# facebookresearch/sam-audio

Hardware: AMD Instinct MI355X
Metric: seconds-of-audio separated/sec/node (higher is better)
Workload: dtype fp16x3 (fp32 storage as the reference; every big contraction on IEEE-half hi + lo split operands: 3 MFMA products per multiply, fp32 accumulation - fp32-grade results on the 16-bit matrix cores)

## Files before the change

### include/samaudio.h

```cpp
#ifndef SAMAUDIO_H_
#define SAMAUDIO_H_

#include <stddef.h>
#include <stdint.h>

#ifdef __cplusplus
extern "C" {
#endif

typedef struct samaudio_ctx samaudio_ctx;
typedef void* samaudio_stream;

enum { SAMAUDIO_F32 = 0, SAMAUDIO_BF16 = 1 };
enum { SAMAUDIO_DT_F32 = 0, SAMAUDIO_DT_BF16 = 1, SAMAUDIO_DT_I64 = 2, SAMAUDIO_DT_U8 = 3 };
enum { SAMAUDIO_ODE_EULER = 0, SAMAUDIO_ODE_MIDPOINT = 1, SAMAUDIO_ODE_RK4 = 2, SAMAUDIO_ODE_HEUN3 = 3 };

enum {
  SAMAUDIO_OK = 0,
  SAMAUDIO_ERR_ARG = -1,
  SAMAUDIO_ERR_WEIGHT = -2,
  SAMAUDIO_ERR_WORKSPACE = -3,
  SAMAUDIO_ERR_HIP = -4,
  SAMAUDIO_ERR_STATE = -5
};
// ... 269 lines not shown
                                      int dim, float eps, samaudio_stream stream);
int samaudio_op_split3(const float* x, int64_t x_ld, void* out, int64_t rows, int k, samaudio_stream stream);


int samaudio_op_mod_tables(const float* const* w, const float* const* shift_tab, const float* const* scale_tab,
                           const int* shift_off, const int* scale_off, int n_norms, const float* tvec, int64_t tvec_ld,
                           int n_time, float* gs, int dim, samaudio_stream stream);
int samaudio_op_rmsnorm_gs(const float* x, const float* gs, int64_t gs_ld, void* out, int precision, int form, int rows,
                           int dim, int rows_per_batch, float eps, samaudio_stream stream);
int samaudio_op_qkv_prep_hd(const void* qkv, const float* q_w, const float* k_w, const float* rope_cos,
                            const float* rope_sin, void* q, void* k, void* vt, int precision, int form, int batch,
                            int frames, int frames_padded, int heads, int head_dim, float eps, samaudio_stream stream);
int samaudio_op_self_attention_hd(const void* q, const void* k, const void* vt, const uint8_t* key_mask, void* out,
                                  int precision, int form, int batch, int frames, int frames_padded, int heads,
                                  int head_dim, samaudio_stream stream);
int samaudio_op_cross_attention_hd(const void* q, const float* q_w, void* kv, int64_t kv_ld, const float* k_w,
                                   const uint8_t* mask, void* out, int precision, int batch, int frames, int text_len,
                                   int heads, int head_dim, float eps, samaudio_stream stream);
int samaudio_op_cross_attn_probs(const void* q, const float* q_w, const void* kv, int64_t kv_ld, const uint8_t* mask, void* p,
                                 int ldp, int batch, int frames, int text_len, int ltp, int heads, float eps,
                                 samaudio_stream stream);
int samaudio_op_cross_attn_probs3(const float* q, const float* q_w, const float* kv, int64_t kv_ld, const uint8_t* mask, void* p3,
                                  int kp, int batch, int frames, int text_len, int ltp, int heads, float eps,
                                  samaudio_stream stream);
int samaudio_op_cross_attn_fold3(const float* wo, const float* kv, int64_t kv_ld, void* ut3, int kp, int batch, int text_len,
                                 int ltp, int heads, samaudio_stream stream);

#ifdef __cplusplus
}
#endif
// ... 2 lines not shown
```

### sam_audio_amd/csrc/api.hip

```cpp
#include <cstring>
#include <string>

#include "engine.h"
#include "peav.h"

struct samaudio_ctx {
  sa::Engine* engine;
};
struct samaudio_judge {
  sa::Judge* judge;
};
struct samaudio_frame {
  sa::FramePredictor* frame;
};

namespace {
thread_local std::string g_err;
}
namespace sa {
void set_last_error(const std::string& msg) { g_err = msg; }
}
namespace {
int hip_ret(hipError_t e, const char* what) {
  if (e == hipSuccess) return SAMAUDIO_OK;
// ... 335 lines not shown
  if (form == 1 && !bf16) return bad("rmsnorm_gs: the alt-16 form belongs to 16-bit contexts");
  return hip_ret(sa::launch_rmsnorm_gs(x, gs, gs_ld, out, bf16, rows, dim, rows_per_batch, eps, (hipStream_t)stream, form == 1),
                 "rmsnorm_gs");
}

int samaudio_op_qkv_prep_hd(const void* qkv, const float* q_w, const float* k_w, const float* rope_cos,
                            const float* rope_sin, void* q, void* k, void* vt, int precision, int form, int batch,
                            int frames, int frames_padded, int heads, int head_dim, float eps, samaudio_stream stream) {
  if (frames_padded % 64 || frames_padded < frames || frames <= 0) return bad("qkv_prep_hd: frames_padded");
  if (head_dim != 64 && head_dim != 128) return bad("qkv_prep_hd: head_dim");
  if (form == 1) {
    if (precision != SAMAUDIO_F32 || head_dim != 128) return bad("qkv_prep_hd: the f32x form takes fp32 tensors and head_dim 128");
    return hip_ret(sa::launch_qkv_prep_f32x((const float*)qkv, q_w, k_w, rope_cos, rope_sin, (float*)q, (float*)k, (float*)vt, batch,
                                            frames, frames_padded, heads, eps, (hipStream_t)stream), "qkv_prep_f32x");
  }
  if (form != 0) return bad("qkv_prep_hd: form");
  return hip_ret(sa::launch_qkv_prep(qkv, q_w, k_w, rope_cos, rope_sin, q, k, vt, precision == SAMAUDIO_BF16, batch, frames,
                                     frames_padded, heads, eps, (hipStream_t)stream, head_dim), "qkv_prep");
}

int samaudio_op_self_attention_hd(const void* q, const void* k, const void* vt, const uint8_t* key_mask, void* out,
                                  int precision, int form, int batch, int frames, int frames_padded, int heads,
                                  int head_dim, samaudio_stream stream) {
  if (frames_padded % 64 || frames_padded < frames || frames <= 0) return bad("self_attention_hd: frames_padded");
  if (head_dim != 64 && head_dim != 128) return bad("self_attention_hd: head_dim");
  if (precision < 0 || precision > 2 || form < 0 || form > 2) return bad("self_attention_hd: precision / form");
  if (form == 1 && precision != SAMAUDIO_BF16) return bad("self_attention_hd: the alt-16 output belongs to the 16-bit kernel");
  if (form == 2 && precision != 2) return bad("self_attention_hd: the split output belongs to the compensated kernel");
  if (precision == 2)
    return hip_ret(sa::launch_self_attention_x3((const float*)q, (const float*)k, (const float*)vt, key_mask,
                                                form == 2 ? nullptr : (float*)out, batch, frames, frames_padded, heads, head_dim,
                                                (hipStream_t)stream, form == 2 ? out : nullptr), "self_attention_x3");
  return hip_ret(sa::launch_self_attention_hd(q, k, vt, key_mask, out, precision == SAMAUDIO_BF16, batch, frames, frames_padded,
                                              heads, head_dim, (hipStream_t)stream, form == 1), "self_attention_hd");
}

int samaudio_op_cross_attention_hd(const void* q, const float* q_w, void* kv, int64_t kv_ld, const float* k_w,
                                   const uint8_t* mask, void* out, int precision, int batch, int frames, int text_len,
                                   int heads, int head_dim, float eps, samaudio_stream stream) {
  if (head_dim != 64 && head_dim != 128) return bad("cross_attention_hd: head_dim");
  if (batch <= 0 || frames <= 0 || text_len <= 0 || heads <= 0 || kv_ld < 2L * heads * head_dim || kv_ld % 8)
    return bad("cross_attention_hd: shape / kv_ld");
  const bool bf16 = precision == SAMAUDIO_BF16;
  hipError_t e = sa::launch_headnorm(kv, k_w, bf16, batch * text_len, kv_ld, 0, heads, eps, (hipStream_t)stream, head_dim);
  if (e != hipSuccess) return hip_ret(e, "headnorm");
  return hip_ret(sa::launch_cross_attention(q, q_w, kv, kv_ld, mask, out, bf16, batch, frames, text_len, heads, eps,
                                            (hipStream_t)stream, head_dim), "cross_attention");
}

int samaudio_op_cross_attn_probs(const void* q, const float* q_w, const void* kv, int64_t kv_ld, const uint8_t* mask, void* p,
                                 int ldp, int batch, int frames, int text_len, int ltp, int heads, float eps,
// ... 122 lines not shown
```

### sam_audio_amd/csrc/attention.hip

```cpp
#include "kernels.h"

namespace sa {

typedef h16x8_t bf16x8_t;
typedef __attribute__((ext_vector_type(4))) float f32x4_t;

template <int NW, int HD, bool OUT_ALT = false>
__global__ __launch_bounds__(NW * 64, 4) void self_attn_bf16_kernel(const bf16_t* __restrict__ Q, const bf16_t* __restrict__ K,
                                                                 const bf16_t* __restrict__ Vt,
                                                                 const unsigned char* __restrict__ key_mask,
                                                                 bf16_t* __restrict__ out, int T, int Tp, int H) {
  constexpr int CH = HD / 8;
  constexpr int KS = HD / 32;
  constexpr int NF = HD / 16;
  __shared__ __attribute__((aligned(16))) char Ks[64 * HD * 2];
  __shared__ __attribute__((aligned(16))) char Vs[HD * 128];
  __shared__ __attribute__((aligned(16))) char Ps[NW * 16 * 128];
  const int qb = blockIdx.x, h = blockIdx.y, b = blockIdx.z;
  const int q0 = qb * (16 * NW);
  const int tid = threadIdx.x, lane = tid & 63, wave = tid >> 6;
  const int lr = lane & 15, lg = lane >> 4;
  const long bh = (long)b * H + h;
  const float scale = HD == 128 ? 0.08838834764831845f : 0.125f;

// ... 399 lines not shown
        bf16_t* dst = out3 + ((long)b * T + q) * (3L * D) + h * HD + c * 8;
        *(uint4*)dst = lo;
        *(uint4*)(dst + D) = hi;
        *(uint4*)(dst + 2L * D) = hi;
      }
    }
    return;
  }
  constexpr int CPRO = HD / 4;
#pragma unroll
  for (int u = lane; u < 16 * CPRO; u += 64) {
    const int row = u / CPRO, c = u % CPRO;
    const int q = q0 + wave * 16 + row;
    if (q < T) *(uint4*)(out + ((long)b * T + q) * D + h * HD + c * 4) = *(const uint4*)(mine + row * (HD * 4) + c * 16);
  }
}

template <int HD>
static hipError_t launch_self_attention_t(const void* Q, const void* K, const void* Vt, const unsigned char* key_mask,
                                          void* out, bool bf16, int B, int T, int Tp, int H, hipStream_t st, bool out_alt = false) {
  if (bf16 && out_alt && Tp % 128 == 0)
    hipLaunchKernelGGL((self_attn_bf16_kernel<8, HD, true>), dim3(Tp / 128, H, B), dim3(512), 0, st, (const bf16_t*)Q, (const bf16_t*)K,
                       (const bf16_t*)Vt, key_mask, (bf16_t*)out, T, Tp, H);
  else if (bf16 && out_alt)
    hipLaunchKernelGGL((self_attn_bf16_kernel<4, HD, true>), dim3(Tp / 64, H, B), dim3(256), 0, st, (const bf16_t*)Q, (const bf16_t*)K,
                       (const bf16_t*)Vt, key_mask, (bf16_t*)out, T, Tp, H);
  else if (out_alt)
    return hipErrorInvalidValue;
  else if (bf16 && Tp % 128 == 0)
    hipLaunchKernelGGL((self_attn_bf16_kernel<8, HD>), dim3(Tp / 128, H, B), dim3(512), 0, st, (const bf16_t*)Q, (const bf16_t*)K,
// ... 605 lines not shown
```

### sam_audio_amd/csrc/engine.h

```cpp
#pragma once
#include "host.h"

namespace sa {

constexpr int HALO = 40;

class Engine {
 public:
  explicit Engine(const samaudio_config& c);
  Status set_tensor(const char* name, const void* p, int dtype, int ndim, const int64_t* shape);
  Status finalize(int what);
  Status set_option(int option, int value);
  Status check_f32_weights(int classes) const;
  size_t workspace_bytes(int rows, int frames, int text_len, int codec_items, int64_t samples);
  Status set_workspace(void* p, size_t bytes);

  Status prepare(int rows, int frames, int text_len, const float* feats, const float* text, const uint8_t* text_mask,
                 const float* video, const int64_t* anchor_ids, int n_ids, const int64_t* anchor_alignment,
                 const uint8_t* pad_mask, hipStream_t st, int candidates = 1, bool latent_feats = false);
  Status forward(const float* noisy, const float* time, int n_time, float* out, hipStream_t st);
  Status ode_solve(float* state, int method, const float* grid_host, int n_grid, hipStream_t st);
  struct RkTableau;
  size_t ode_stage_bytes(int method, int rows, int frames) const;
  Status set_ode_stages(void* p, size_t bytes);
// ... 44 lines not shown
  bool f32c(int cls) const { return bf16_ && (f32_classes_ & cls) != 0; }
  bool alt16(int cls) const { return bf16_ && (alt_classes_ & cls) != 0; }
  const void* opt(const std::string& name, std::vector<int64_t> shape) const;
  struct ProfRec {
    std::string key;
    double flops, bytes;
    hipEvent_t e0, e1;
  };
  template <class F>
  Status op(const char* name, double alg_bytes, double alg_flops, hipStream_t st, F&& launch);
  Status res_unit(GemmParams p, GemmParams q, void*& cur, void*& alt, double flops7, double flops1, hipStream_t st);
  struct SBuf;
  struct StageW;
  Status res_units(const StageW& sw, SBuf& sb, int n, const float* next_alpha, hipStream_t st);
  void* hash_ = nullptr;
  bool prof_on_ = false;
  std::vector<ProfRec> prof_;
  std::vector<hipEvent_t> ev_pool_;
  size_t ev_used_ = 0;
  Status prof_event(hipEvent_t* e);

  samaudio_config cfg_;
  bool bf16_;
  bool tail_split_ = true;
  int f32_classes_ = 0;
  int alt_classes_ = 0;
  int prefetch_rows_ = 0;
  int x3_classes_ = 0;
  Status solve_launches(float* y, int method, const float* grid, int n_grid, hipStream_t st);
  Status solve_rk(float* y, const RkTableau& tab, const float* grid, int n_grid, hipStream_t st);
// ... 62 lines not shown
```

### sam_audio_amd/csrc/engine.hip

```cpp
#include "engine.h"

#include <algorithm>
#include <cmath>
#include <cstdio>
#include <cstdlib>
#include <cstring>

namespace sa {

static bool trace_on() {
  static const bool on = std::getenv("SAMAUDIO_TRACE") != nullptr;
  return on;
}
struct HashTrace {
  struct Rec { std::string name; int items; size_t slot; };
  unsigned long long* dev = nullptr;
  size_t used = 0, seq = 0;
  std::vector<Rec> recs;
  static constexpr size_t CAP = 1 << 20;
  bool full_warned = false;
};
struct HashScope {
  explicit HashScope(HashTrace* h, int items);
  ~HashScope();
// ... 55 lines not shown
#else
      const unsigned u = (unsigned)((const unsigned short*)host.data())[i] << 16;
      std::memcpy(&v, &u, 4);
#endif
    } else {
      v = ((const float*)host.data())[i];
    }
    if (!std::isfinite(v)) ++bad;
    else if (std::fabs(v) > mx) mx = std::fabs(v);
  }
  std::fprintf(stderr, "[samaudio trace] %-22s n=%zu non-finite=%zu max|x|=%.4g\n", name, count, bad, mx);
}

Engine::Engine(const samaudio_config& c) : cfg_(c) {
  bf16_ = c.precision == SAMAUDIO_BF16;
  esz_ = bf16_ ? 2 : 4;
  at_dtype_ = bf16_ ? SAMAUDIO_DT_BF16 : SAMAUDIO_DT_F32;
  std::memset(&g32_, 0, sizeof(g32_));
  std::memset(&enc_, 0, sizeof(enc_));
  std::memset(&dec_, 0, sizeof(dec_));
  std::memset(&d_, 0, sizeof(d_));
}

Status Registry::set(const char* name, const void* p, int dtype, int ndim, const int64_t* shape) {
  if (!name || !p || ndim < 0 || ndim > 4) return fail(SAMAUDIO_ERR_ARG, "set_tensor: bad argument");
  if ((reinterpret_cast<uintptr_t>(p) & 15) != 0)
    return fail(SAMAUDIO_ERR_ARG, std::string("set_tensor: ") + name + " is not 16-byte aligned");
  TensorRef t;
  t.p = p;
  t.dtype = dtype;
// ... 1004 lines not shown
    return p;
  };
  for (int l = 0; l < cfg_.n_layers; ++l) {
    const LayerW& w = layers_[l];
    const float* tab = w.mod_table;
    const bool qkv_pre = x3(SAMAUDIO_CLS_QKV) && mod_gs, w13_pre = x3(SAMAUDIO_CLS_W13) && mod_gs;
    const bool wo_pre = x3(SAMAUDIO_CLS_WO) && x3(SAMAUDIO_X3_ATTENTION);
    bool w2_pre = false;
    SA_TRY(norm_for(l, 0, SAMAUDIO_CLS_QKV, qkv_pre));
    {
      GemmParams p = lin(d_.xn, D, nullptr, M, 3 * D, D);
      prefetch(p, w.wo.w, (double)D * D);
      out_act(p, d_.qkv, 3L * D);
      SA_TRY(linear(p, w.wqkv, SAMAUDIO_CLS_QKV, st, qkv_pre ? d_.x3a : nullptr));
    }
    SA_TRY(op("qkv_prep", 2 * 3 * MD * esz_, 0, st, [&] {
      if (x3(SAMAUDIO_X3_ATTENTION) && hd == 128)
        return launch_qkv_prep_f32x((const float*)d_.qkv, w.q_norm, w.k_norm, g_.rope_cos, g_.rope_sin, (float*)d_.Q, (float*)d_.K,
                                    (float*)d_.Vt, rows, T, Tp, H, eps, st);
      return launch_qkv_prep(d_.qkv, w.q_norm, w.k_norm, g_.rope_cos, g_.rope_sin, d_.Q, d_.K, d_.Vt, bf16_, rows, T, Tp, H,
                             eps, st, hd);
    }));
    trace("  xn", d_.xn, (size_t)M * D, bf16_, st);
    trace("  qkv", d_.qkv, (size_t)M * 3 * D, bf16_, st);
    trace("  Q", d_.Q, (size_t)rows * Tp * D, bf16_, st);
    trace("  K", d_.K, (size_t)rows * Tp * D, bf16_, st);
    trace("  Vt", d_.Vt, (size_t)rows * Tp * D, bf16_, st);
    if (x3(SAMAUDIO_X3_ATTENTION))
      SA_TRY(op("self_attention_x3", 4 * MD * 4, 4.0 * T * T * D * rows, st, [&] {
        return launch_self_attention_x3((const float*)d_.Q, (const float*)d_.K, (const float*)d_.Vt, d_.pad_mask, (float*)d_.attn, rows,
                                        T, Tp, H, hd, st, wo_pre ? d_.x3a : nullptr);
      }));
    else
    SA_TRY(op("self_attention", 4 * MD * esz_, 4.0 * T * T * D * rows, st, [&] {
      return launch_self_attention_hd(d_.Q, d_.K, d_.Vt, d_.pad_mask, d_.attn, bf16_, rows, T, Tp, H, hd, st, alt16(SAMAUDIO_CLS_WO));
    }));
    trace("  attn", d_.attn, (size_t)M * D, bf16_, st);
    SA_TRY(sentinel(15, d_.attn, !bf16_ ? 0 : (alt16(SAMAUDIO_CLS_WO) ? 2 : 1), M, D, D, st));
    {
      GemmParams p = lin(d_.attn, D, nullptr, M, D, D);
      p.gate_tab = tab + 2 * D; p.gate = d_.t0 + 2 * D; p.gate_ld = t6; p.rows_per_gate = T;
      with_res(p, d_.h, D);
      out_f32(p, d_.h, D);
      out_act(p, d_.hbf, D);
// ... 370 lines not shown
```

### sam_audio_amd/csrc/kernels.h

```cpp
#pragma once
#include "common.h"

namespace sa {

hipError_t launch_poison_lds(hipStream_t st);

enum DebugFlag : int {
  DBG_NO_CONV7H = 11,
  DBG_RESUNIT_TWO_LAUNCHES = 16,
  DBG_RESUNIT_FUSE_ALWAYS = 18,
  DBG_RESUNIT_WS = 19,
  DBG_GEMM8S_PLAIN = 21,
  DBG_GEMM8_EPILOGUE = 24,
  DBG_GEMM8_NOT_PERSISTENT = 26,
  DBG_GEMM8S_ROLES = 27,
  DBG_QKV_PREP_SWROUND = 29,
  DBG_GEMM8_MIN_TILES = 30,
  DBG_FOLD_PER_LAYER = 31,
  DBG_TAIL_SPLIT_MIN = 33,
  DBG_RASTER_GM = 35,
  DBG_FLY_OLD_TILES = 36,
  DBG_X3_PLAIN_WALK = 38,
};
enum : int { DBG_WS_ALWAYS = 1, DBG_WS_NEVER = 2, DBG_WS_ALWAYS_GRID3 = 3 };
// ... 108 lines not shown
                           float eps, hipStream_t st, int head_dim = 128);

hipError_t launch_qkv_prep_f32x(const float* qkv, const float* qw, const float* kw, const float* rope_cos, const float* rope_sin, float* Q,
                                float* K, float* Vt, int B, int T, int Tp, int H, float eps, hipStream_t st);

hipError_t launch_self_attention(const void* Q, const void* K, const void* Vt, const unsigned char* key_mask,
                                 void* out, bool bf16, int B, int T, int Tp, int H, hipStream_t st, bool out_alt = false);

hipError_t launch_self_attention_hd(const void* Q, const void* K, const void* Vt, const unsigned char* key_mask,
                                    void* out, bool bf16, int B, int T, int Tp, int H, int head_dim, hipStream_t st,
                                    bool out_alt = false);

hipError_t launch_self_attention_x3(const float* Q, const float* K, const float* Vt, const unsigned char* key_mask, float* out,
                                    int B, int T, int Tp, int H, int head_dim, hipStream_t st, void* out3 = nullptr);

hipError_t launch_headnorm(void* x, const float* w, bool bf16, int rows, long ld, int col0, int H, float eps,
                           hipStream_t st, int head_dim = 128);

hipError_t launch_cross_attention(const void* q, const float* qw, const void* kv, long kv_ld,
                                  const unsigned char* mask, void* out, bool bf16, int B, int T, int Lt, int H,
                                  float eps, hipStream_t st, int head_dim = 128);
hipError_t launch_cross_attn_probs(const void* q, const float* qw, const void* kv, long kv_ld, const unsigned char* mask,
                                   void* P, int ldp, int B, int T, int Lt, int LtP, int H, float eps, hipStream_t st);
hipError_t launch_cross_attn_fold(const void* wo, const void* kv, long kv_ld, void* UT, int KP, int B, int Lt, int LtP,
                                  int H, hipStream_t st);
constexpr int kMaxFoldLayers = 48;
hipError_t launch_cross_attn_fold_layers(const void* const* wo, int n_layers, const void* kv_all, long kv_ld, void* UT_all, int KP,
                                         int B, int Lt, int LtP, int H, hipStream_t st);
hipError_t launch_cross_attn_probs3(const float* q, const float* qw, const float* kv, long kv_ld, const unsigned char* mask, void* P3,
                                    int KP, int B, int T, int Lt, int LtP, int H, float eps, hipStream_t st);
// ... 83 lines not shown
```

### sam_audio_amd/csrc/kernels.hip

```cpp
#include "kernels.h"

namespace sa {

static int g_debug_flags[64] = {0};
void set_debug_flag(int flag, int value) {
  if (flag >= 0 && flag < 64) g_debug_flags[flag] = value;
}
int debug_flag(int flag) { return flag >= 0 && flag < 64 ? g_debug_flags[flag] : 0; }

template <typename TO>
__global__ __launch_bounds__(256) void rmsnorm_mod_kernel(const float* __restrict__ x, const float* __restrict__ w,
                                                          const float* __restrict__ shift_tab,
                                                          const float* __restrict__ scale_tab,
                                                          const float* __restrict__ tvec, long tvec_ld, int shift_off,
                                                          int scale_off, TO* __restrict__ out, int M, int D,
                                                          int rows_per_b, float eps) {
  const int row = blockIdx.x * 4 + (threadIdx.x >> 6);
  if (row >= M) return;
  const int lane = threadIdx.x & 63;
  const float4* xr = (const float4*)(x + (long)row * D);
  const int n4 = D >> 2;
  float ss = 0.f;
  for (int i = lane; i < n4; i += 64) {
    float4 v = xr[i];
// ... 427 lines not shown
  }
  __syncthreads();
#pragma unroll
  for (int it = 0; it < 4; ++it) {
    const int item = it * 256 + tid;
    const int d = item >> 3, c = item & 7;
    unsigned short x[8];
#pragma unroll
    for (int e = 0; e < 8; ++e) x[e] = vt[(c * 8 + e) * 136 + d];
    const uint4 o = make_uint4((unsigned)x[0] | ((unsigned)x[1] << 16), (unsigned)x[2] | ((unsigned)x[3] << 16),
                               (unsigned)x[4] | ((unsigned)x[5] << 16), (unsigned)x[6] | ((unsigned)x[7] << 16));
    *(uint4*)(Vt + (bh * 128 + d) * Tp + t0 + c * 8) = o;
  }
}

__global__ __launch_bounds__(256) void qkv_prep_f32x_kernel(const float* __restrict__ qkv, const float* __restrict__ qw,
                                                            const float* __restrict__ kw, const float* __restrict__ rc,
                                                            const float* __restrict__ rs, float* __restrict__ Q, float* __restrict__ K,
                                                            float* __restrict__ Vt, int T, int Tp, int H, float eps) {
  __shared__ __attribute__((aligned(16))) float vt[64 * 132];
  const int t0 = blockIdx.x * 64, h = blockIdx.y, b = blockIdx.z;
  const int D = H * 128;
  const long ld = 3L * D;
  const int tid = threadIdx.x;
  const int sub = tid & 15;
  const int rgrp = tid >> 4;
  const long bh = (long)b * H + h;
  float wq[8], wk[8];
  {
    const float4 a = *(const float4*)(qw + sub * 8), c = *(const float4*)(qw + sub * 8 + 4);
    const float4 e = *(const float4*)(kw + sub * 8), f = *(const float4*)(kw + sub * 8 + 4);
    wq[0] = a.x; wq[1] = a.y; wq[2] = a.z; wq[3] = a.w; wq[4] = c.x; wq[5] = c.y; wq[6] = c.z; wq[7] = c.w;
    wk[0] = e.x; wk[1] = e.y; wk[2] = e.z; wk[3] = e.w; wk[4] = f.x; wk[5] = f.y; wk[6] = f.z; wk[7] = f.w;
  }
#pragma unroll
// ... 15 lines not shown
      sq = row16_sum(sq);
      sk = row16_sum(sk);
      const float iq = rsqrtf(sq / 128.f + eps), ik = rsqrtf(sk / 128.f + eps);
      const float4 c4 = *(const float4*)(rc + (long)t * 64 + sub * 4), s4 = *(const float4*)(rs + (long)t * 64 + sub * 4);
      const float cc[4] = {c4.x, c4.y, c4.z, c4.w}, sn[4] = {s4.x, s4.y, s4.z, s4.w};
#pragma unroll
      for (int e = 0; e < 4; ++e) {
        const float a0 = q[2 * e] * iq * wq[2 * e], a1 = q[2 * e + 1] * iq * wq[2 * e + 1];
        q[2 * e] = a0 * cc[e] - a1 * sn[e];
        q[2 * e + 1] = a0 * sn[e] + a1 * cc[e];
        const float b0 = k[2 * e] * ik * wk[2 * e], b1 = k[2 * e + 1] * ik * wk[2 * e + 1];
        k[2 * e] = b0 * cc[e] - b1 * sn[e];
        k[2 * e + 1] = b0 * sn[e] + b1 * cc[e];
      }
    }
    float* qd = Q + (bh * Tp + t) * 128 + sub * 8;
    float* kd = K + (bh * Tp + t) * 128 + sub * 8;
    *(float4*)qd = make_float4(q[0], q[1], q[2], q[3]);
    *(float4*)(qd + 4) = make_float4(q[4], q[5], q[6], q[7]);
    *(float4*)kd = make_float4(k[0], k[1], k[2], k[3]);
    *(float4*)(kd + 4) = make_float4(k[4], k[5], k[6], k[7]);
    *(float4*)(vt + tt * 132 + sub * 8) = v0;
    *(float4*)(vt + tt * 132 + sub * 8 + 4) = v1;
  }
  __syncthreads();
#pragma unroll
  for (int it = 0; it < 4; ++it) {
    const int item = it * 256 + tid;
    const int d = item >> 3, c = item & 7;
    float x[8];
#pragma unroll
    for (int e = 0; e < 8; ++e) x[e] = vt[(c * 8 + e) * 132 + d];
    float* dst = Vt + (bh * 128 + d) * Tp + t0 + c * 8;
    *(float4*)dst = make_float4(x[0], x[1], x[2], x[3]);
    *(float4*)(dst + 4) = make_float4(x[4], x[5], x[6], x[7]);
  }
}
hipError_t launch_qkv_prep_f32x(const float* qkv, const float* qw, const float* kw, const float* rope_cos, const float* rope_sin, float* Q,
                                float* K, float* Vt, int B, int T, int Tp, int H, float eps, hipStream_t st) {
  if (Tp % 64) return hipErrorInvalidValue;
  hipLaunchKernelGGL(qkv_prep_f32x_kernel, dim3(Tp / 64, H, B), dim3(256), 0, st, qkv, qw, kw, rope_cos, rope_sin, Q, K, Vt, T, Tp, H, eps);
  return hipGetLastError();
}

hipError_t launch_qkv_prep(const void* qkv, const float* qw, const float* kw, const float* rope_cos,
                           const float* rope_sin, void* Q, void* K, void* Vt, bool bf16, int B, int T, int Tp, int H,
                           float eps, hipStream_t st, int head_dim) {
  dim3 grid(Tp / 64, H, B), block(256);
  if (head_dim == 64) {
    if (bf16)
      hipLaunchKernelGGL((qkv_prep_kernel<bf16_t, 64>), grid, block, 0, st, (const bf16_t*)qkv, qw, kw, rope_cos, rope_sin, (bf16_t*)Q,
                         (bf16_t*)K, (bf16_t*)Vt, T, Tp, H, eps);
    else
      hipLaunchKernelGGL((qkv_prep_kernel<float, 64>), grid, block, 0, st, (const float*)qkv, qw, kw, rope_cos, rope_sin, (float*)Q,
                         (float*)K, (float*)Vt, T, Tp, H, eps);
    return hipGetLastError();
// ... 506 lines not shown
```

### sam_audio_amd/hip.py

```python
from __future__ import annotations

import ctypes as C
import os
import threading
from typing import Optional, Sequence

_HERE = os.path.dirname(os.path.abspath(__file__))
LIB_PATH = os.path.join(_HERE, "libsamaudio_hip.so")
LIB_PATHS = {"bf16": LIB_PATH, "fp16": os.path.join(_HERE, "libsamaudio_hip_f16.so")}

F32, BF16 = 0, 1
DT_F32, DT_BF16, DT_I64, DT_U8 = 0, 1, 2, 3
PRECISIONS = ("bf16", "fp16", "mixed", "fp32")
X3_PRECISIONS = ("fp16x3", "bf16x3")


def check_precision(precision: str, x3_ok: bool = False) -> None:
    if precision not in PRECISIONS + (X3_PRECISIONS if x3_ok else ()):
        raise ValueError("precision must be 'bf16', 'fp16', 'mixed' or 'fp32'" + (", 'fp16x3' or 'bf16x3'" if x3_ok else ""))


def is_x3(precision: str) -> bool:
    return precision in X3_PRECISIONS

# ... 226 lines not shown
    "samaudio_op_self_attention": (C.c_int, [C.c_void_p] * 5 + [C.c_int] * 5 + [C.c_void_p]),
    "samaudio_op_cross_attention": (C.c_int, [C.c_void_p] * 6 + [C.c_int] * 5 + [C.c_float, C.c_void_p]),
    "samaudio_op_cross_attn_fold": (C.c_int, [C.c_void_p, C.c_void_p, C.c_int64, C.c_void_p] + [C.c_int] * 5 + [C.c_void_p]),
    "samaudio_op_layernorm_accum": (C.c_int, [C.c_void_p] * 5 + [C.c_int, C.c_int, C.c_float, C.c_void_p]),
    "samaudio_op_masked_groupnorm_silu": (C.c_int, [C.c_void_p] * 6 + [C.c_int] * 5 + [C.c_float, C.c_void_p]),
    "samaudio_op_masked_groupnorm_silu_split3": (C.c_int, [C.c_void_p] * 6 + [C.c_int] * 4 + [C.c_float, C.c_void_p]),
    "samaudio_op_layernorm_rows": (C.c_int, [C.c_void_p, C.c_int64] + [C.c_void_p] * 4 + [C.c_int, C.c_int64, C.c_int,
                                                                                          C.c_float, C.c_void_p]),
    "samaudio_op_layernorm_rows_split3": (C.c_int, [C.c_void_p, C.c_int64] + [C.c_void_p] * 3 + [C.c_int64, C.c_int, C.c_float, C.c_void_p]),
    "samaudio_op_split3": (C.c_int, [C.c_void_p, C.c_int64, C.c_void_p, C.c_int64, C.c_int, C.c_void_p]),
    "samaudio_op_mod_tables": (C.c_int, [C.POINTER(C.c_void_p)] * 3 + [C.POINTER(C.c_int)] * 2 + [C.c_int, C.c_void_p, C.c_int64,
                                                                                                 C.c_int, C.c_void_p, C.c_int, C.c_void_p]),
    "samaudio_op_rmsnorm_gs": (C.c_int, [C.c_void_p, C.c_void_p, C.c_int64, C.c_void_p] + [C.c_int] * 5 + [C.c_float, C.c_void_p]),
    "samaudio_op_qkv_prep_hd": (C.c_int, [C.c_void_p] * 8 + [C.c_int] * 7 + [C.c_float, C.c_void_p]),
    "samaudio_op_self_attention_hd": (C.c_int, [C.c_void_p] * 5 + [C.c_int] * 7 + [C.c_void_p]),
    "samaudio_op_cross_attention_hd": (C.c_int, [C.c_void_p] * 3 + [C.c_int64] + [C.c_void_p] * 3 + [C.c_int] * 6 + [C.c_float, C.c_void_p]),
    "samaudio_op_cross_attn_probs": (C.c_int, [C.c_void_p] * 3 + [C.c_int64, C.c_void_p, C.c_void_p] + [C.c_int] * 6 + [C.c_float, C.c_void_p]),
    "samaudio_op_cross_attn_probs3": (C.c_int, [C.c_void_p] * 3 + [C.c_int64, C.c_void_p, C.c_void_p] + [C.c_int] * 6 + [C.c_float, C.c_void_p]),
    "samaudio_op_cross_attn_fold3": (C.c_int, [C.c_void_p, C.c_void_p, C.c_int64, C.c_void_p] + [C.c_int] * 5 + [C.c_void_p]),
    "samaudio_judge_create": (C.c_int, [C.POINTER(JudgeConfig), C.POINTER(C.c_void_p)]),
    "samaudio_judge_destroy": (None, [C.c_void_p]),
    "samaudio_judge_set_tensor": (C.c_int, [C.c_void_p, C.c_char_p, C.c_void_p, C.c_int, C.c_int, C.POINTER(C.c_int64)]),
    "samaudio_judge_set_option": (C.c_int, [C.c_void_p, C.c_int, C.c_int]),
    "samaudio_judge_finalize": (C.c_int, [C.c_void_p]),
    "samaudio_judge_workspace_bytes": (C.c_size_t, [C.c_void_p, C.c_int, C.c_int, C.c_int]),
    "samaudio_judge_set_workspace": (C.c_int, [C.c_void_p, C.c_void_p, C.c_size_t]),
    "samaudio_judge_score": (C.c_int, [C.c_void_p, C.c_void_p, C.c_void_p, C.c_int, C.c_int, C.c_int, C.c_void_p,
                                       C.c_void_p, C.c_void_p, C.c_void_p]),
    "samaudio_judge_encode": (C.c_int, [C.c_void_p, C.c_int, C.c_void_p, C.c_void_p, C.c_int, C.c_int, C.c_void_p,
                                        C.c_void_p]),
# ... 101 lines not shown
```

Measured before the change: 95.23.

## Pre-split Q/K/V into hi/lo 16-bit planes for compensated self-attention

The qkv prep kernel gains a planes mode that writes Q, K and V^T as separate high and low 16-bit planes instead of fp32. A new self-attention kernel reads these planes directly, staging K and V^T in LDS through register prefetch, and runs the three-product split MFMAs without re-splitting fp32 operands inside the loop. The goal is to halve attention operand traffic and remove the per-tile split work. It adds weak-symbol dispatch and an environment opt-out, and it depends on the split done at prep time matching the accuracy of the old path.

```diff
diff --git a/include/samaudio.h b/include/samaudio.h
--- a/include/samaudio.h
+++ b/include/samaudio.h
@@ -307,6 +307,8 @@
 int samaudio_op_self_attention_hd(const void* q, const void* k, const void* vt, const uint8_t* key_mask, void* out,
                                   int precision, int form, int batch, int frames, int frames_padded, int heads,
                                   int head_dim, samaudio_stream stream);
+int samaudio_op_self_attention_planes(const void* q, const void* k, const void* vt, const uint8_t* key_mask, void* out, int form,
+                                      int batch, int frames, int frames_padded, int heads, samaudio_stream stream);
 int samaudio_op_cross_attention_hd(const void* q, const float* q_w, void* kv, int64_t kv_ld, const float* k_w,
                                    const uint8_t* mask, void* out, int precision, int batch, int frames, int text_len,
                                    int heads, int head_dim, float eps, samaudio_stream stream);
diff --git a/sam_audio_amd/csrc/api.hip b/sam_audio_amd/csrc/api.hip
--- a/sam_audio_amd/csrc/api.hip
+++ b/sam_audio_amd/csrc/api.hip
@@ -373,6 +373,17 @@
     return hip_ret(sa::launch_qkv_prep_f32x((const float*)qkv, q_w, k_w, rope_cos, rope_sin, (float*)q, (float*)k, (float*)vt, batch,
                                             frames, frames_padded, heads, eps, (hipStream_t)stream), "qkv_prep_f32x");
   }
+  if (form == 2) {
+    if (precision != SAMAUDIO_F32 || head_dim != 128) return bad("qkv_prep_hd: the planes form takes fp32 tensors and head_dim 128");
+    if (!qkv || !q_w || !k_w || !rope_cos || !rope_sin || !q || !k || !vt || batch <= 0 || heads <= 0)
+      return bad("qkv_prep_hd: null argument / batch, heads");
+    if (!sa::launch_qkv_prep_planes) {
+      g_err = "qkv_prep_hd: the planes form is not in this build of the library";
+      return SAMAUDIO_ERR_STATE;
+    }
+    return hip_ret(sa::launch_qkv_prep_planes((const float*)qkv, q_w, k_w, rope_cos, rope_sin, q, k, vt, batch, frames, frames_padded,
+                                              heads, eps, (hipStream_t)stream), "qkv_prep_planes");
+  }
   if (form != 0) return bad("qkv_prep_hd: form");
   return hip_ret(sa::launch_qkv_prep(qkv, q_w, k_w, rope_cos, rope_sin, q, k, vt, precision == SAMAUDIO_BF16, batch, frames,
                                      frames_padded, heads, eps, (hipStream_t)stream, head_dim), "qkv_prep");
@@ -394,6 +405,19 @@
                                               heads, head_dim, (hipStream_t)stream, form == 1), "self_attention_hd");
 }
 
+int samaudio_op_self_attention_planes(const void* q, const void* k, const void* vt, const uint8_t* key_mask, void* out, int form,
+                                      int batch, int frames, int frames_padded, int heads, samaudio_stream stream) {
+  if (!q || !k || !vt || !key_mask || !out || batch <= 0 || heads <= 0) return bad("self_attention_planes: null argument / batch, heads");
+  if (frames_padded % 64 || frames_padded < frames || frames <= 0) return bad("self_attention_planes: frames_padded");
+  if (form != 0 && form != 2) return bad("self_attention_planes: form");
+  if (!sa::launch_self_attention_x3p) {
+    g_err = "self_attention_planes: not in this build of the library";
+    return SAMAUDIO_ERR_STATE;
+  }
+  return hip_ret(sa::launch_self_attention_x3p(q, k, vt, key_mask, form == 2 ? nullptr : (float*)out, batch, frames, frames_padded, heads,
+                                               (hipStream_t)stream, form == 2 ? out : nullptr), "self_attention_x3p");
+}
+
 int samaudio_op_cross_attention_hd(const void* q, const float* q_w, void* kv, int64_t kv_ld, const float* k_w,
                                    const uint8_t* mask, void* out, int precision, int batch, int frames, int text_len,
                                    int heads, int head_dim, float eps, samaudio_stream stream) {
diff --git a/sam_audio_amd/csrc/attention.hip b/sam_audio_amd/csrc/attention.hip
--- a/sam_audio_amd/csrc/attention.hip
+++ b/sam_audio_amd/csrc/attention.hip
@@ -437,6 +437,273 @@
     const int q = q0 + wave * 16 + row;
     if (q < T) *(uint4*)(out + ((long)b * T + q) * D + h * HD + c * 4) = *(const uint4*)(mine + row * (HD * 4) + c * 16);
   }
+}
+
+typedef __attribute__((ext_vector_type(4))) unsigned u32x4_t;
+template <int NW, int RB, bool OUT3>
+__global__ __launch_bounds__(NW * 64) void self_attn_x3p_kernel(const bf16_t* __restrict__ Q, const bf16_t* __restrict__ K,
+                                                                const bf16_t* __restrict__ Vt,
+                                                                const unsigned char* __restrict__ key_mask, float* __restrict__ out,
+                                                                bf16_t* __restrict__ out3, int T, int Tp, int H) {
+  constexpr int HD = 128, KS = HD / 32, NF = HD / 16;
+  constexpr int KB = 64 * HD * 2;
+  constexpr int MAXT = 2048;
+  constexpr int KS_ = 0, VS_ = 2 * KB, PS_ = 4 * KB, PL = NW * RB * 2048, MS_ = PS_ + 2 * PL;
+  __shared__ __attribute__((aligned(16))) char smem[MS_ + MAXT];
+  const int h = blockIdx.y, b = blockIdx.z;
+  const int q0 = blockIdx.x * (16 * NW * RB);
+  const int tid = threadIdx.x, lane = tid & 63, wave = tid >> 6;
+  const int lr = lane & 15, lg = lane >> 4;
+  const long bh = (long)b * H + h;
+  const long plane = (long)gridDim.z * H * Tp * HD;
+  const float scale = 0.08838834764831845f;
+
+  bf16x8_t qh[RB][KS], ql[RB][KS];
+#pragma unroll
+  for (int rb = 0; rb < RB; ++rb) {
+    const bf16_t* qrow = Q + (bh * Tp + q0 + (wave * RB + rb) * 16 + lr) * HD;
+#pragma unroll
+    for (int ks = 0; ks < KS; ++ks) {
+      qh[rb][ks] = *(const bf16x8_t*)(qrow + (ks * 4 + lg) * 8);
+      ql[rb][ks] = *(const bf16x8_t*)(qrow + plane + (ks * 4 + lg) * 8);
+    }
+  }
+  const bool mask_in_lds = Tp <= MAXT;
+  if (mask_in_lds)
+    for (int i = tid; i < Tp; i += NW * 64) smem[MS_ + i] = (i < T && key_mask[(long)b * T + (i < T ? i : 0)] != 0) ? 1 : 0;
+  float m_i[RB][4], l_i[RB][4];
+  f32x4_t o[RB][NF];
+#pragma unroll
+  for (int rb = 0; rb < RB; ++rb) {
+#pragma unroll
+    for (int r = 0; r < 4; ++r) { m_i[rb][r] = -INFINITY; l_i[rb][r] = 0.f; }
+#pragma unroll
+    for (int n = 0; n < NF; ++n) o[rb][n] = f32x4_t{0.f, 0.f, 0.f, 0.f};
+  }
+  const bool odd = (lr & 1) != 0;
+  const int pw = PS_ + wave * (RB * 2048);
+  int kfrag[KS], vfrag[2], pfrag[2], pst[2][2];
+#pragma unroll
+  for (int ks = 0; ks < KS; ++ks) kfrag[ks] = KS_ + lr * (HD * 2) + (((ks * 4 + lg) ^ lr) << 4);
+#pragma unroll
+  for (int ks = 0; ks < 2; ++ks) {
+    vfrag[ks] = VS_ + lr * 128 + (((ks * 4 + lg) ^ ((lr >> 1) & 7)) << 4);
+    pfrag[ks] = pw + lr * 128 + (((ks * 4 + lg) ^ ((lr >> 1) & 7)) << 4);
+  }
+#pragma unroll
+  for (int a = 0; a < 2; ++a)
+#pragma unroll
+    for (int rh = 0; rh < 2; ++rh) {
+      const int c = (2 * a + (odd ? 1 : 0)) * 2 + (lr >> 3), sw = (lg * 2 + rh) & 7;
+      pst[a][rh] = pw + lg * 512 + ((c ^ sw) << 4) + ((lr & 7) >> 1) * 4;
+    }
+  int kst = KS_ + (tid >> 4) * (HD * 2) + (((tid & 15) ^ ((tid >> 4) & 15)) << 4);
+  int vst = VS_ + (tid >> 3) * 128 + (((tid & 7) ^ ((tid >> 4) & 7)) << 4);
+  int msk = MS_ + lr;
+
+  constexpr int NIT = 1024 / (64 * NW);
+  u32x4_t stage[NIT][2];
+  const bf16_t* const Kbh = K + bh * Tp * HD;
+  const bf16_t* const Vbh = Vt + bh * HD * Tp;
+  const unsigned koff = tid * 8, voff = (tid >> 3) * Tp + (tid & 7) * 8;
+  auto request_k = [&](int kt) {
+    const bf16_t* base = Kbh + (long)kt * HD;
+#pragma unroll
+    for (int it = 0; it < NIT; ++it) {
+      stage[it][0] = *(const u32x4_t*)(base + it * (64 * NW * 8) + koff);
+      stage[it][1] = *(const u32x4_t*)(base + plane + it * (64 * NW * 8) + koff);
+    }
+  };
+  auto request_v = [&](int kt) {
+#pragma unroll
+    for (int it = 0; it < NIT; ++it) {
+      const bf16_t* base = Vbh + (long)it * (8 * NW) * Tp + kt;
+      stage[it][0] = *(const u32x4_t*)(base + voff);
+      stage[it][1] = *(const u32x4_t*)(base + plane + voff);
+    }
+  };
+  request_k(0);
+  __syncthreads();
+  for (int kt = 0; kt < Tp; kt += 64) {
+#pragma unroll
+    for (int ks = 0; ks < KS; ++ks) asm volatile("" : "+v"(kfrag[ks]));
+#pragma unroll
+    for (int ks = 0; ks < 2; ++ks) {
+      asm volatile("" : "+v"(vfrag[ks]));
+      asm volatile("" : "+v"(pfrag[ks]));
+      asm volatile("" : "+v"(pst[ks][0]));
+      asm volatile("" : "+v"(pst[ks][1]));
+    }
+    asm volatile("" : "+v"(kst));
+    asm volatile("" : "+v"(vst));
+    asm volatile("" : "+v"(msk));
+#pragma unroll
+    for (int it = 0; it < NIT; ++it) {
+      *(u32x4_t*)(smem + (kst + it * (NW * 1024))) = stage[it][0];
+      *(u32x4_t*)(smem + (kst + it * (NW * 1024) + KB)) = stage[it][1];
+    }
+    request_v(kt);
+    __syncthreads();
+    f32x4_t s[RB][4];
+#pragma unroll
+    for (int nb = 0; nb < 4; ++nb) {
+#pragma unroll
+      for (int rb = 0; rb < RB; ++rb) s[rb][nb] = f32x4_t{0.f, 0.f, 0.f, 0.f};
+#pragma unroll
+      for (int ks = 0; ks < KS; ++ks) {
+        const bf16x8_t kh = *(const bf16x8_t*)(smem + (kfrag[ks] + nb * 4096)), kl = *(const bf16x8_t*)(smem + (kfrag[ks] + nb * 4096 + KB));
+#pragma unroll
+        for (int rb = 0; rb < RB; ++rb) {
+          s[rb][nb] = SA_MFMA_16x16x32(ql[rb][ks], kh, s[rb][nb]);
+          s[rb][nb] = SA_MFMA_16x16x32(qh[rb][ks], kl, s[rb][nb]);
+        }
+      }
+#pragma unroll
+      for (int ks = 0; ks < KS; ++ks) {
+        const bf16x8_t kh = *(const bf16x8_t*)(smem + (kfrag[ks] + nb * 4096));
+#pragma unroll
+        for (int rb = 0; rb < RB; ++rb) s[rb][nb] = SA_MFMA_16x16x32(qh[rb][ks], kh, s[rb][nb]);
+      }
+    }
+    bool valid[4];
+#pragma unroll
+    for (int nb = 0; nb < 4; ++nb) {
+      const int key = kt + nb * 16 + lr;
+      valid[nb] = mask_in_lds ? smem[msk + kt + nb * 16] != 0 : (key < T && key_mask[(long)b * T + key] != 0);
+    }
+#pragma unroll
+    for (int rb = 0; rb < RB; ++rb) {
+#pragma unroll
+      for (int r = 0; r < 4; ++r) {
+        float mx = -INFINITY;
+#pragma unroll
+        for (int nb = 0; nb < 4; ++nb) {
+          s[rb][nb][r] = valid[nb] ? s[rb][nb][r] * scale : -INFINITY;
+          mx = fmaxf(mx, s[rb][nb][r]);
+        }
+        mx = row16_max(mx);
+        const float m_new = fmaxf(m_i[rb][r], mx);
+        const float m_safe = m_new == -INFINITY ? 0.f : m_new;
+        const float alpha = expf(m_i[rb][r] - m_safe);
+        float rs = 0.f;
+#pragma unroll
+        for (int nb = 0; nb < 4; ++nb) {
+          const float pv = expf(s[rb][nb][r] - m_safe);
+          s[rb][nb][r] = pv;
+          rs += pv;
+        }
+        rs = row16_sum(rs);
+        l_i[rb][r] = l_i[rb][r] * alpha + rs;
+        m_i[rb][r] = m_new;
+#pragma unroll
+        for (int n = 0; n < NF; ++n) o[rb][n][r] *= alpha;
+        unsigned w[4];
+#pragma unroll
+        for (int nb = 0; nb < 4; ++nb) {
+          const unsigned short ph = f2bf(s[rb][nb][r]);
+          w[nb] = (unsigned)ph | ((unsigned)f2bf(s[rb][nb][r] - bf2f(ph)) << 16);
+        }
+#pragma unroll
+        for (int a = 0; a < 2; ++a) {
+          const float x = __uint_as_float(odd ? w[2 * a] : w[2 * a + 1]);
+          const unsigned from_left = __float_as_uint(dpp_mov<0x121>(x)), from_right = __float_as_uint(dpp_mov<0x12F>(x));
+          const unsigned first = odd ? from_left : w[2 * a], second = odd ? w[2 * a + 1] : from_right;
+          const int at = pst[a][r >> 1] + r * 128 + rb * 2048;
+          *(unsigned*)(smem + at) = (first & 0xffffu) | (second << 16);
+          *(unsigned*)(smem + (at + PL)) = (first >> 16) | (second & 0xffff0000u);
+        }
+      }
+    }
+#pragma unroll
+    for (int it = 0; it < NIT; ++it) {
+      *(u32x4_t*)(smem + (vst + it * (NW * 1024))) = stage[it][0];
+      *(u32x4_t*)(smem + (vst + it * (NW * 1024) + KB)) = stage[it][1];
+    }
+    if (kt + 64 < Tp) request_k(kt + 64);
+    __syncthreads();
+#pragma unroll
+    for (int ks = 0; ks < 2; ++ks) {
+      bf16x8_t ph[RB], pl[RB];
+#pragma unroll
+      for (int rb = 0; rb < RB; ++rb) {
+        ph[rb] = *(const bf16x8_t*)(smem + (pfrag[ks] + rb * 2048));
+        pl[rb] = *(const bf16x8_t*)(smem + (pfrag[ks] + rb * 2048 + PL));
+      }
+#pragma unroll
+      for (int n = 0; n < NF; ++n) {
+        const bf16x8_t vh = *(const bf16x8_t*)(smem + (vfrag[ks] + n * 2048)), vl = *(const bf16x8_t*)(smem + (vfrag[ks] + n * 2048 + KB));
+#pragma unroll
+        for (int rb = 0; rb < RB; ++rb) {
+          o[rb][n] = SA_MFMA_16x16x32(pl[rb], vh, o[rb][n]);
+          o[rb][n] = SA_MFMA_16x16x32(ph[rb], vl, o[rb][n]);
+          o[rb][n] = SA_MFMA_16x16x32(ph[rb], vh, o[rb][n]);
+        }
+      }
+    }
+  }
+  const int D = H * HD;
+  __syncthreads();
+  constexpr int SLICE = 16 * HD * 4;
+  static_assert(NW * SLICE <= 4 * KB, "output staging fits the K / V^T staging areas");
+  char* mine = smem + wave * SLICE;
+#pragma unroll
+  for (int rb = 0; rb < RB; ++rb) {
+    const int qw0 = q0 + (wave * RB + rb) * 16;
+#pragma unroll
+    for (int r = 0; r < 4; ++r) {
+      const float inv = 1.f / l_i[rb][r];
+      const int q = lg * 4 + r;
+#pragma unroll
+      for (int n = 0; n < NF; ++n) *(float*)(mine + q * (HD * 4) + (n * 16 + lr) * 4) = o[rb][n][r] * inv;
+    }
+    asm volatile("s_waitcnt lgkmcnt(0)" ::: "memory");
+    if constexpr (OUT3) {
+      constexpr int CPR8 = HD / 8;
+#pragma unroll
+      for (int u = lane; u < 16 * CPR8; u += 64) {
+        const int row = u / CPR8, c = u % CPR8;
+        const int q = qw0 + row;
+        const float* src = (const float*)(mine + row * (HD * 4) + c * 32);
+        uint4 hi, lo;
+        split8(*(const float4*)src, *(const float4*)(src + 4), hi, lo);
+        if (q < T) {
+          bf16_t* dst = out3 + ((long)b * T + q) * (3L * D) + h * HD + c * 8;
+          *(uint4*)dst = lo;
+          *(uint4*)(dst + D) = hi;
+          *(uint4*)(dst + 2L * D) = hi;
+        }
+      }
+    } else {
+      constexpr int CPRO = HD / 4;
+#pragma unroll
+      for (int u = lane; u < 16 * CPRO; u += 64) {
+        const int row = u / CPRO, c = u % CPRO;
+        const int q = qw0 + row;
+        if (q < T) *(uint4*)(out + ((long)b * T + q) * D + h * HD + c * 4) = *(const uint4*)(mine + row * (HD * 4) + c * 16);
+      }
+    }
+    if (rb + 1 < RB) asm volatile("s_waitcnt lgkmcnt(0)" ::: "memory");
+  }
+}
+
+template <int NW, int RB>
+static void launch_self_attention_x3p_t(const void* Q, const void* K, const void* Vt, const unsigned char* key_mask, float* out, void* out3,
+                                        int B, int T, int Tp, int H, hipStream_t st) {
+  const dim3 grid(Tp / (16 * NW * RB), H, B);
+  if (out3)
+    hipLaunchKernelGGL((self_attn_x3p_kernel<NW, RB, true>), grid, dim3(NW * 64), 0, st, (const bf16_t*)Q, (const bf16_t*)K,
+                       (const bf16_t*)Vt, key_mask, out, (bf16_t*)out3, T, Tp, H);
+  else
+    hipLaunchKernelGGL((self_attn_x3p_kernel<NW, RB, false>), grid, dim3(NW * 64), 0, st, (const bf16_t*)Q, (const bf16_t*)K,
+                       (const bf16_t*)Vt, key_mask, out, (bf16_t*)nullptr, T, Tp, H);
+}
+hipError_t launch_self_attention_x3p(const void* Q, const void* K, const void* Vt, const unsigned char* key_mask, float* out, int B, int T,
+                                     int Tp, int H, hipStream_t st, void* out3) {
+  if (Tp % 64 || (!out && !out3)) return hipErrorInvalidValue;
+  if (Tp % 256 == 0 && (long)(Tp / 256) * H * B >= 256) launch_self_attention_x3p_t<8, 2>(Q, K, Vt, key_mask, out, out3, B, T, Tp, H, st);
+  else if (Tp % 128 == 0) launch_self_attention_x3p_t<8, 1>(Q, K, Vt, key_mask, out, out3, B, T, Tp, H, st);
+  else launch_self_attention_x3p_t<4, 1>(Q, K, Vt, key_mask, out, out3, B, T, Tp, H, st);
+  return hipGetLastError();
 }
 
 template <int HD>
diff --git a/sam_audio_amd/csrc/engine.h b/sam_audio_amd/csrc/engine.h
--- a/sam_audio_amd/csrc/engine.h
+++ b/sam_audio_amd/csrc/engine.h
@@ -82,6 +82,7 @@
   struct StageW;
   Status res_units(const StageW& sw, SBuf& sb, int n, const float* next_alpha, hipStream_t st);
   void* hash_ = nullptr;
+  bool attn_planes_ = false;
   bool prof_on_ = false;
   std::vector<ProfRec> prof_;
   std::vector<hipEvent_t> ev_pool_;
diff --git a/sam_audio_amd/csrc/engine.hip b/sam_audio_amd/csrc/engine.hip
--- a/sam_audio_amd/csrc/engine.hip
+++ b/sam_audio_amd/csrc/engine.hip
@@ -93,6 +93,7 @@
 
 Engine::Engine(const samaudio_config& c) : cfg_(c) {
   bf16_ = c.precision == SAMAUDIO_BF16;
+  attn_planes_ = launch_qkv_prep_planes && launch_self_attention_x3p && std::getenv("SAMAUDIO_NO_SPLIT_ATTENTION") == nullptr;
   esz_ = bf16_ ? 2 : 4;
   at_dtype_ = bf16_ ? SAMAUDIO_DT_BF16 : SAMAUDIO_DT_F32;
   std::memset(&g32_, 0, sizeof(g32_));
@@ -1127,7 +1128,11 @@
       out_act(p, d_.qkv, 3L * D);
       SA_TRY(linear(p, w.wqkv, SAMAUDIO_CLS_QKV, st, qkv_pre ? d_.x3a : nullptr));
     }
+    const bool planes = attn_planes_ && x3(SAMAUDIO_X3_ATTENTION) && hd == 128;
     SA_TRY(op("qkv_prep", 2 * 3 * MD * esz_, 0, st, [&] {
+      if (planes)
+        return launch_qkv_prep_planes((const float*)d_.qkv, w.q_norm, w.k_norm, g_.rope_cos, g_.rope_sin, d_.Q, d_.K, d_.Vt, rows, T, Tp,
+                                      H, eps, st);
       if (x3(SAMAUDIO_X3_ATTENTION) && hd == 128)
         return launch_qkv_prep_f32x((const float*)d_.qkv, w.q_norm, w.k_norm, g_.rope_cos, g_.rope_sin, (float*)d_.Q, (float*)d_.K,
                                     (float*)d_.Vt, rows, T, Tp, H, eps, st);
@@ -1141,6 +1146,8 @@
     trace("  Vt", d_.Vt, (size_t)rows * Tp * D, bf16_, st);
     if (x3(SAMAUDIO_X3_ATTENTION))
       SA_TRY(op("self_attention_x3", 4 * MD * 4, 4.0 * T * T * D * rows, st, [&] {
+        if (planes)
+          return launch_self_attention_x3p(d_.Q, d_.K, d_.Vt, d_.pad_mask, (float*)d_.attn, rows, T, Tp, H, st, wo_pre ? d_.x3a : nullptr);
         return launch_self_attention_x3((const float*)d_.Q, (const float*)d_.K, (const float*)d_.Vt, d_.pad_mask, (float*)d_.attn, rows,
                                         T, Tp, H, hd, st, wo_pre ? d_.x3a : nullptr);
       }));
diff --git a/sam_audio_amd/csrc/kernels.h b/sam_audio_amd/csrc/kernels.h
--- a/sam_audio_amd/csrc/kernels.h
+++ b/sam_audio_amd/csrc/kernels.h
@@ -146,6 +146,12 @@
 hipError_t launch_self_attention_x3(const float* Q, const float* K, const float* Vt, const unsigned char* key_mask, float* out,
                                     int B, int T, int Tp, int H, int head_dim, hipStream_t st, void* out3 = nullptr);
 
+__attribute__((weak)) hipError_t launch_qkv_prep_planes(const float* qkv, const float* qw, const float* kw, const float* rope_cos,
+                                                        const float* rope_sin, void* Q, void* K, void* Vt, int B, int T, int Tp, int H,
+                                                        float eps, hipStream_t st);
+__attribute__((weak)) hipError_t launch_self_attention_x3p(const void* Q, const void* K, const void* Vt, const unsigned char* key_mask,
+                                                           float* out, int B, int T, int Tp, int H, hipStream_t st, void* out3 = nullptr);
+
 hipError_t launch_headnorm(void* x, const float* w, bool bf16, int rows, long ld, int col0, int H, float eps,
                            hipStream_t st, int head_dim = 128);
 
diff --git a/sam_audio_amd/csrc/kernels.hip b/sam_audio_amd/csrc/kernels.hip
--- a/sam_audio_amd/csrc/kernels.hip
+++ b/sam_audio_amd/csrc/kernels.hip
@@ -465,11 +465,19 @@
   }
 }
 
+template <bool PLANES = false>
 __global__ __launch_bounds__(256) void qkv_prep_f32x_kernel(const float* __restrict__ qkv, const float* __restrict__ qw,
                                                             const float* __restrict__ kw, const float* __restrict__ rc,
                                                             const float* __restrict__ rs, float* __restrict__ Q, float* __restrict__ K,
                                                             float* __restrict__ Vt, int T, int Tp, int H, float eps) {
   __shared__ __attribute__((aligned(16))) float vt[64 * 132];
+  const long plane = (long)gridDim.z * H * Tp * 128;
+  auto split_store = [plane](float* base, long at, const float (&x)[8]) {
+    const H16Split s0 = split_h16x2(x[0], x[1]), s1 = split_h16x2(x[2], x[3]), s2 = split_h16x2(x[4], x[5]), s3 = split_h16x2(x[6], x[7]);
+    bf16_t* hi = (bf16_t*)base + at;
+    *(uint4*)hi = make_uint4(s0.hi, s1.hi, s2.hi, s3.hi);
+    *(uint4*)(hi + plane) = make_uint4(s0.lo, s1.lo, s2.lo, s3.lo);
+  };
   const int t0 = blockIdx.x * 64, h = blockIdx.y, b = blockIdx.z;
   const int D = H * 128;
   const long ld = 3L * D;
@@ -515,12 +523,17 @@
         k[2 * e + 1] = b0 * sn[e] + b1 * cc[e];
       }
     }
-    float* qd = Q + (bh * Tp + t) * 128 + sub * 8;
-    float* kd = K + (bh * Tp + t) * 128 + sub * 8;
-    *(float4*)qd = make_float4(q[0], q[1], q[2], q[3]);
-    *(float4*)(qd + 4) = make_float4(q[4], q[5], q[6], q[7]);
-    *(float4*)kd = make_float4(k[0], k[1], k[2], k[3]);
-    *(float4*)(kd + 4) = make_float4(k[4], k[5], k[6], k[7]);
+    if constexpr (PLANES) {
+      split_store(Q, (bh * Tp + t) * 128 + sub * 8, q);
+      split_store(K, (bh * Tp + t) * 128 + sub * 8, k);
+    } else {
+      float* qd = Q + (bh * Tp + t) * 128 + sub * 8;
+      float* kd = K + (bh * Tp + t) * 128 + sub * 8;
+      *(float4*)qd = make_float4(q[0], q[1], q[2], q[3]);
+      *(float4*)(qd + 4) = make_float4(q[4], q[5], q[6], q[7]);
+      *(float4*)kd = make_float4(k[0], k[1], k[2], k[3]);
+      *(float4*)(kd + 4) = make_float4(k[4], k[5], k[6], k[7]);
+    }
     *(float4*)(vt + tt * 132 + sub * 8) = v0;
     *(float4*)(vt + tt * 132 + sub * 8 + 4) = v1;
   }
@@ -532,15 +545,26 @@
     float x[8];
 #pragma unroll
     for (int e = 0; e < 8; ++e) x[e] = vt[(c * 8 + e) * 132 + d];
-    float* dst = Vt + (bh * 128 + d) * Tp + t0 + c * 8;
-    *(float4*)dst = make_float4(x[0], x[1], x[2], x[3]);
-    *(float4*)(dst + 4) = make_float4(x[4], x[5], x[6], x[7]);
+    if constexpr (PLANES) {
+      split_store(Vt, (bh * 128 + d) * Tp + t0 + c * 8, x);
+    } else {
+      float* dst = Vt + (bh * 128 + d) * Tp + t0 + c * 8;
+      *(float4*)dst = make_float4(x[0], x[1], x[2], x[3]);
+      *(float4*)(dst + 4) = make_float4(x[4], x[5], x[6], x[7]);
+    }
   }
 }
 hipError_t launch_qkv_prep_f32x(const float* qkv, const float* qw, const float* kw, const float* rope_cos, const float* rope_sin, float* Q,
                                 float* K, float* Vt, int B, int T, int Tp, int H, float eps, hipStream_t st) {
   if (Tp % 64) return hipErrorInvalidValue;
-  hipLaunchKernelGGL(qkv_prep_f32x_kernel, dim3(Tp / 64, H, B), dim3(256), 0, st, qkv, qw, kw, rope_cos, rope_sin, Q, K, Vt, T, Tp, H, eps);
+  hipLaunchKernelGGL(qkv_prep_f32x_kernel<false>, dim3(Tp / 64, H, B), dim3(256), 0, st, qkv, qw, kw, rope_cos, rope_sin, Q, K, Vt, T, Tp, H, eps);
+  return hipGetLastError();
+}
+hipError_t launch_qkv_prep_planes(const float* qkv, const float* qw, const float* kw, const float* rope_cos, const float* rope_sin, void* Q,
+                                  void* K, void* Vt, int B, int T, int Tp, int H, float eps, hipStream_t st) {
+  if (Tp % 64) return hipErrorInvalidValue;
+  hipLaunchKernelGGL(qkv_prep_f32x_kernel<true>, dim3(Tp / 64, H, B), dim3(256), 0, st, qkv, qw, kw, rope_cos, rope_sin, (float*)Q, (float*)K,
+                     (float*)Vt, T, Tp, H, eps);
   return hipGetLastError();
 }
 
diff --git a/sam_audio_amd/hip.py b/sam_audio_amd/hip.py
--- a/sam_audio_amd/hip.py
+++ b/sam_audio_amd/hip.py
@@ -264,6 +264,7 @@
     "samaudio_op_rmsnorm_gs": (C.c_int, [C.c_void_p, C.c_void_p, C.c_int64, C.c_void_p] + [C.c_int] * 5 + [C.c_float, C.c_void_p]),
     "samaudio_op_qkv_prep_hd": (C.c_int, [C.c_void_p] * 8 + [C.c_int] * 7 + [C.c_float, C.c_void_p]),
     "samaudio_op_self_attention_hd": (C.c_int, [C.c_void_p] * 5 + [C.c_int] * 7 + [C.c_void_p]),
+    "samaudio_op_self_attention_planes": (C.c_int, [C.c_void_p] * 5 + [C.c_int] * 5 + [C.c_void_p]),
     "samaudio_op_cross_attention_hd": (C.c_int, [C.c_void_p] * 3 + [C.c_int64] + [C.c_void_p] * 3 + [C.c_int] * 6 + [C.c_float, C.c_void_p]),
     "samaudio_op_cross_attn_probs": (C.c_int, [C.c_void_p] * 3 + [C.c_int64, C.c_void_p, C.c_void_p] + [C.c_int] * 6 + [C.c_float, C.c_void_p]),
     "samaudio_op_cross_attn_probs3": (C.c_int, [C.c_void_p] * 3 + [C.c_int64, C.c_void_p, C.c_void_p] + [C.c_int] * 6 + [C.c_float, C.c_void_p]),
```

After: 95.89 (median of 6 runs). Within noise of the previous version (+0.7%).
